# toybox-rs/Toybox

Hardware: NVIDIA B200
Metric: env-steps/sec with rendered frames (higher is better)
Workload: dtype f64+u8

## Files before the change

### toybox_b200/csrc/tbx_direct.cu

```cuda
#include <mutex>
#include "tbx_render_direct.cuh"
#include <stdlib.h>
#include <vector>

using namespace tbxk;

static int align16(int v) { return (v + 15) & ~15; }

template <class D> static cudaError_t upload_direct(const std::vector<D> &A, Buf<uint8_t> &aux) {
  return A[0].ok ? aux.upload(reinterpret_cast<const uint8_t *>(A.data()), sizeof(D)) : cudaSuccess;
}

cudaError_t tbx_direct_build(const tbx::Config &c, const BrkTable *brk_default, const tbx::ResizeTab &rs, const TbxAreaPlan &plan, const uint8_t *base0_gray,
                             Buf<uint8_t> &aux, Buf<uint8_t> &aux2) {
  if (c.game == TBX_BREAKOUT) {
    if (!brk_default) return cudaSuccess;
    std::vector<TbxBrkDirect> A(1);
    tbx::build_brk_direct(c, *brk_default, rs, plan, base0_gray, A[0]);
    return upload_direct(A, aux);
  }
  if (c.game == TBX_AMIDAR) {
    std::vector<TbxAmiDirect> A(1);
    tbx::build_ami_direct(c, rs, plan, A[0]);
    return upload_direct(A, aux);
  }
  std::vector<TbxSiDirect> A(1);
  std::vector<TbxSpritePatch> patches;
  tbx::build_si_direct(c, rs, plan, base0_gray, A[0], patches);
  const cudaError_t e = upload_direct(A, aux);
  if (e != cudaSuccess || !aux || patches.empty()) return e;
  return aux2.upload(reinterpret_cast<const uint8_t *>(patches.data()), patches.size() * sizeof(TbxSpritePatch));
}

template <class K> static cudaError_t persistent_grid(K kernel, int smem, int n_chunks, int *grid_out) {
  struct Entry { const void *k; int smem, dev, resident; };
  static Entry cache[64];
  static int n_cache = 0;
  static std::mutex mu;
  int dev = 0;
  cudaGetDevice(&dev);
  int resident = 0;
  {
    std::lock_guard<std::mutex> lock(mu);
    for (int i = 0; i < n_cache; i++)
      if (cache[i].k == (const void *)kernel && cache[i].smem == smem && cache[i].dev == dev) resident = cache[i].resident;
  }
  if (!resident) {
    int per_sm = 0, sms = 0;
    cudaError_t e = cudaOccupancyMaxActiveBlocksPerMultiprocessor(&per_sm, kernel, TBX_DIRECT_THREADS, smem);
    if (e != cudaSuccess) return e;
    cudaDeviceGetAttribute(&sms, cudaDevAttrMultiProcessorCount, dev);
    resident = (per_sm > 0 ? per_sm : 1) * (sms > 0 ? sms : 148);
    std::lock_guard<std::mutex> lock(mu);
    if (n_cache < 64) cache[n_cache++] = Entry{(const void *)kernel, smem, dev, resident};
  }
  int grid = n_chunks < resident ? n_chunks : resident;
  if (const char *env = getenv("TBX_DIRECT_GRID")) if (atoi(env) > 0) grid = atoi(env) < n_chunks ? atoi(env) : n_chunks;
  *grid_out = grid;
  return cudaSuccess;
}

template <class... P, class... A> static cudaError_t launch_persistent(void (*kernel)(P...), int smem, int n, cudaStream_t s, const A &...args) {
  cudaError_t e = cudaFuncSetAttribute(kernel, cudaFuncAttributeMaxDynamicSharedMemorySize, smem);
  if (e != cudaSuccess) return e;
  int grid = 1;
  e = persistent_grid(kernel, smem, (n + TBX_EPC - 1) / TBX_EPC, &grid);
  if (e != cudaSuccess) return e;
  kernel<<<grid, TBX_DIRECT_THREADS, smem, s>>>(args...);
  return cudaGetLastError();
}

cudaError_t tbx_launch_direct(const tbx::Config &c, const RenderArgs &a, const TbxAreaPlan &plan, DirectArgs d, cudaStream_t s) {
// ... 40 lines not shown
```

### toybox_b200/csrc/tbx_direct.h

```cpp
#ifndef TBX_DIRECT_H
#define TBX_DIRECT_H
#include "tbx_breakout.h"
#include "tbx_space_invaders.h"
#include "tbx_amidar.h"

struct TbxMover { int x0, y0, x1, y1; uint32_t gray; };

#define TBX_BD_MAX_STATIC 16
#define TBX_BD_MAX_CLS 8
#define BRK_N_MOVERS (1 + TBX_BRK_MAX_BALLS)
typedef struct TbxBrkDirect {
  int32_t ok;
  int32_t ncols, nrows;
  int32_t wx0, wy0, bw, bh;
  int32_t wdy0, wdy1;
  int32_t hud_dyhi;
  int32_t n_static, _pad;
  uint32_t paddle_gray, ball_gray;
  uint8_t xcol[TBX_AREA_MAX_SRC];
  uint8_t yrow[TBX_AREA_MAX_SRC];
  uint8_t col0[TBX_AREA_MAX_DST];
  uint8_t dyrows[TBX_AREA_MAX_DST];
  uint8_t hsel[TBX_AREA_MAX_DST][TBX_AREA_MAX_TAPS];
  uint32_t wordcols[32];
  uint8_t brickgray[TBX_BRK_MAX_BRICKS];
  uint32_t inv32[TBX_AREA_MAX_DST + 1];
  alignas(16) float hlut[TBX_BRK_MAX_ROWS][4][TBX_AREA_MAX_DST];
  alignas(16) float hstatic[TBX_BD_MAX_STATIC][TBX_AREA_MAX_DST];
  int32_t n_cls, _pad2[3];
  uint8_t rowcls[TBX_BRK_H];
  alignas(16) uint8_t clsrows[TBX_BD_MAX_CLS * TBX_BRK_W + 16];
} TbxBrkDirect;

TBX_HD TbxMover brk_mover(const uint32_t *R, const BrkCfg &c, uint32_t paddle_gray, uint32_t ball_gray, int m) {
  TbxMover v; v.x0 = v.y0 = v.x1 = v.y1 = 0; v.gray = m == 0 ? paddle_gray : ball_gray;
  if (m < 0 || m >= BRK_N_MOVERS) return v;
  const TbxPrim p = brk_prim(R, c, (const BrkTable *)0, m == 0 ? BRK_SLOT_PADDLE : BRK_SLOT_BALLS + m - 1);
  if (p.h <= 0) return v;
  const int x0 = p.x < 0 ? 0 : p.x, y0 = p.y < 0 ? 0 : p.y;
  const int x1 = p.x + p.w > TBX_BRK_W ? TBX_BRK_W : p.x + p.w, y1 = p.y + p.h > TBX_BRK_H ? TBX_BRK_H : p.y + p.h;
  if (x0 >= x1 || y0 >= y1) return v;
  v.x0 = x0; v.y0 = y0; v.x1 = x1; v.y1 = y1;
  return v;
}

TBX_HD uint32_t brk_col_bits(const uint32_t *alive, int nrows, int c) {
  const int i0 = c * nrows, w = i0 >> 5, s = i0 & 31;
  const uint32_t lo = alive[w], hi = w < 4 ? alive[w + 1] : 0u;
  const uint32_t v = s ? (lo >> s) | (hi << (32 - s)) : lo;
  return v & ((1u << nrows) - 1u);
}

TBX_HD uint32_t brk_direct_src(const TbxBrkDirect &A, const uint8_t *base0, const uint32_t *alive, const TbxMover *mv, uint32_t near, bool wall,
                               int x, int y) {
  uint32_t v = base0[y * TBX_BRK_W + x];
  if (wall) {
    const uint32_t c = A.xcol[x], r = A.yrow[y];
    if ((c | r) != 255u) {
      const uint32_t i = c * (uint32_t)A.nrows + r;
      if ((alive[i >> 5] >> (i & 31)) & 1u) v = A.brickgray[i];
    }
  }
#if defined(__CUDA_ARCH__)
#pragma unroll
#endif
  for (int m = 0; m < BRK_N_MOVERS; m++)
    if ((near >> m) & 1u)
      if ((unsigned)(x - mv[m].x0) < (unsigned)(mv[m].x1 - mv[m].x0) && (unsigned)(y - mv[m].y0) < (unsigned)(mv[m].y1 - mv[m].y0)) v = mv[m].gray;
  return v;
}

template <int TX, int TY>
TBX_HD uint8_t brk_direct_pixel(const TbxBrkDirect &A, const TbxAreaPlan &pl, const uint8_t *base0, const uint32_t *alive, const TbxMover *mv, uint32_t near,
                                bool wall, int dx, int dy) {
  const int xs = pl.xs0[dx], ys = pl.ys0[dy];
  float acc = 0.0f;
#if defined(__CUDA_ARCH__)
#pragma unroll
#endif
  for (int k = 0; k < TY; k++) {
    const int y = ys + k < TBX_BRK_H ? ys + k : TBX_BRK_H - 1;
    float h = 0.0f;
#if defined(__CUDA_ARCH__)
#pragma unroll
#endif
// ... 87 lines not shown
```

### toybox_b200/csrc/tbx_host.cpp

```cpp
#include "tbx_host.h"
#include "tbx_breakout.h"
#include "tbx_space_invaders.h"
#include "tbx_amidar.h"
#include "tbx_direct.h"
#include <errno.h>
#include <math.h>
#include <string.h>

using tbxjson::Value;

namespace tbx {

static void fail(const std::string &m) { throw std::runtime_error(m); }

static const GameInfo GAMES[3] = {
    {TBX_BREAKOUT, "breakout", TBX_BRK_W, TBX_BRK_H, 4, {0, 1, 3, 4}, TBX_WORDS(BrkRec), BRK_N_SLOTS, 2},
    {TBX_AMIDAR, "amidar", TBX_AMI_W, TBX_AMI_H, 10, {0, 1, 2, 3, 4, 5, 10, 11, 12, 13}, TBX_WORDS(AmiRec), AMI_N_SLOTS, 1},
    {TBX_SPACE_INVADERS, "space_invaders", TBX_SI_W, TBX_SI_H, 6, {0, 1, 3, 4, 11, 12}, TBX_WORDS(SiRec), SI_N_SLOTS, 2},
};
const GameInfo *game_info(int game) { return game >= 0 && game < 3 ? &GAMES[game] : 0; }
int game_from_name(const char *name) {
  if (!name) return -1;
  for (int g = 0; g < 3; g++) if (strcmp(GAMES[g].name, name) == 0) return g;
  if (strcmp(name, "spaceinvaders") == 0) return TBX_SPACE_INVADERS;
// ... 844 lines not shown
  for (int y = 0; y < H; y++) for (int dx = 0; dx < dw; dx++) buf[(size_t)y * dw + dx] = tbx_area_h(gray + (size_t)y * W, t.x, dx);
  for (int dy = 0; dy < dh; dy++) for (int dx = 0; dx < dw; dx++) out[dy * dw + dx] = tbx_area_v(buf.data(), dw, 0, t.y, dy, dx);
}
int digit_slot0(int game) { return game == TBX_BREAKOUT ? BRK_SLOT_SCORE : game == TBX_AMIDAR ? AMI_SLOT_SCORE : SI_SLOT_SCORE; }
int digit_slots(int game) { return game == TBX_BREAKOUT ? BRK_SLOT_BRICKS - BRK_SLOT_SCORE : game == TBX_AMIDAR ? AMI_N_SLOTS - AMI_SLOT_SCORE : SI_SLOT_SHIELDS - SI_SLOT_SCORE; }
static uint8_t area_pixel(const uint8_t *gray, int W, const ResizeTab &t, int dx, int dy) {
  int k = t.y.start[dy], k1 = t.y.start[dy + 1];
  float s = tbx_fmul(t.y.alpha[k], tbx_area_h(gray + (size_t)t.y.si[k] * W, t.x, dx));
  for (k++; k < k1; k++) s = tbx_fadd(s, tbx_fmul(t.y.alpha[k], tbx_area_h(gray + (size_t)t.y.si[k] * W, t.x, dx)));
  int v = tbx_f2i_rn(s);
  return (uint8_t)(v < 0 ? 0 : v > 255 ? 255 : v);
}
void build_digit_patches(const Config &c, const BrkTable *brk_default, const ResizeTab &t, const TbxAreaPlan &plan, const uint8_t *base_gray,
                         TbxDigitPatch *out) {
  const GameInfo *gi = game_info(c.game);
  const int W = gi->width, H = gi->height;
  std::vector<uint8_t> gray(base_gray, base_gray + (size_t)W * H);
  std::vector<uint32_t> rec(gi->rec_words, 0);
  memset(out, 0, sizeof(TbxDigitPatch) * TBX_DP_SLOTS * 10);
  const int s0 = digit_slot0(c.game), ns = digit_slots(c.game);
  for (int idx = 0; idx < ns && idx < TBX_DP_SLOTS; idx++) {
    const int k = idx % TBX_MAX_DIGITS;
    for (int d = 0; d < 10; d++) {
      long long v = d;
      for (int i = 0; i < k; i++) v *= 10;
      if (d == 0 && k > 0) { v = 1; for (int i = 0; i <= k; i++) v *= 10; }
      if (v > 2000000000LL) continue;
      std::fill(rec.begin(), rec.end(), 0u);
      TbxHdr &h = *reinterpret_cast<TbxHdr *>(rec.data());
      h.score = (int32_t)v; h.lives = (int32_t)v;
      TbxPrim p;
      if (c.game == TBX_BREAKOUT) p = brk_prim(rec.data(), c.brk, brk_default, s0 + idx);
      else if (c.game == TBX_AMIDAR) { reinterpret_cast<AmiRec *>(rec.data())->jumps = (int32_t)v; p = ami_prim(rec.data(), c.ami, 0, s0 + idx); }
      else { reinterpret_cast<SiRec *>(rec.data())->life_display_timer = 1; p = si_prim(rec.data(), s0 + idx); }
      if (p.h <= 0 || p.bw != 3 || p.off != TBX_BANK_FONT + 5 * d) continue;
      const int x0 = p.x < 0 ? 0 : p.x, x1 = p.x + p.w > W ? W : p.x + p.w, y0 = p.y < 0 ? 0 : p.y, y1 = p.y + p.h > H ? H : p.y + p.h;
      if (x0 >= x1 || y0 >= y1) continue;
      const int dx0 = plan.xdlo[x0], dx1 = plan.xdhi[x1 - 1], dy0 = plan.ydlo[y0], dy1 = plan.ydhi[y1 - 1];
      const int w = dx1 - dx0 + 1, hh = dy1 - dy0 + 1;
      if (w < 1 || hh < 1 || w > 8 || w * hh > TBX_DP_MAX) continue;
      const uint8_t lum = (uint8_t)tbx_luma(p.color);
      for (int y = y0; y < y1; y++)
        for (int x = x0; x < x1; x++)
          if (tbx_prim_covers(p, HOST_BANK, rec.data(), x, y)) gray[(size_t)y * W + x] = lum;
      TbxDigitPatch &P = out[idx * 10 + d];
      P.x0 = (uint8_t)dx0; P.y0 = (uint8_t)dy0; P.w = (uint8_t)w; P.h = (uint8_t)hh;
      for (int r = 0; r < hh; r++)
        for (int cc = 0; cc < w; cc++) P.px[r * w + cc] = area_pixel(gray.data(), W, t, dx0 + cc, dy0 + r);
      for (int y = y0; y < y1; y++) memcpy(&gray[(size_t)y * W + x0], base_gray + (size_t)y * W + x0, (size_t)(x1 - x0));
    }
  }
}

static float hsum_row(const uint8_t *row, int W, const TbxAreaPlan &pl, int dx) {
  float h = 0.0f;
  for (int t = 0; t < TBX_AREA_MAX_TAPS; t++) {
    const int x = pl.xs0[dx] + t < W ? pl.xs0[dx] + t : W - 1;
    const float p = tbx_fmul((float)row[x], pl.xalpha[t][dx]);
    h = t == 0 ? p : tbx_fadd(h, p);
  }
  return h;
}
void build_brk_direct(const Config &c, const BrkTable &t, const ResizeTab &rs, const TbxAreaPlan &pl, const uint8_t *base0, TbxBrkDirect &A) {
  memset(&A, 0, sizeof A);
  const int W = TBX_BRK_W, H = TBX_BRK_H, dw = pl.dw, dh = pl.dh;
  if (c.game != TBX_BREAKOUT || !t.delta_ok || dw % 4 != 0 || dw > TBX_AREA_MAX_DST || dh > TBX_AREA_MAX_DST || pl.tx > 5 || pl.ty > 4) return;
  const int n = t.n_bricks, nrows = c.brk.n_rows;
  if (n <= 0 || nrows <= 0 || nrows > TBX_BRK_MAX_ROWS || n % nrows != 0) return;
  const int ncols = n / nrows;
  if (ncols > 31) return;
  const int bw = t.iw[0], bh = t.ih[0], wx0 = t.ix[0], wy0 = t.iy[0];
  if (bw <= 0 || bh <= 0 || wx0 < 0 || wy0 < 0 || wx0 + ncols * bw > W || wy0 + nrows * bh > H) return;
  for (int i = 0; i < n; i++) {
    const int col = i / nrows, row = i % nrows;
    if (t.ix[i] != wx0 + col * bw || t.iy[i] != wy0 + row * bh || t.iw[i] != bw || t.ih[i] != bh) return;
    A.brickgray[i] = (uint8_t)tbx_luma(t.color[i]);
  }
  A.ncols = ncols; A.nrows = nrows; A.wx0 = wx0; A.wy0 = wy0; A.bw = bw; A.bh = bh;
  A.paddle_gray = tbx_luma(c.brk.paddle_color); A.ball_gray = tbx_luma(c.brk.ball_color);
  for (int k = 2; k <= TBX_AREA_MAX_DST; k++) A.inv32[k] = 0xffffffffu / (uint32_t)k + 1u;
  memset(A.xcol, 255, sizeof A.xcol);
  memset(A.yrow, 255, sizeof A.yrow);
  for (int x = wx0; x < wx0 + ncols * bw; x++) A.xcol[x] = (uint8_t)((x - wx0) / bw);
  for (int y = wy0; y < wy0 + nrows * bh; y++) A.yrow[y] = (uint8_t)((y - wy0) / bh);
  for (int r = 0; r < nrows; r++)
    for (int y = wy0 + r * bh + 1; y < wy0 + (r + 1) * bh; y++)
      if (memcmp(base0 + (size_t)y * W, base0 + (size_t)(wy0 + r * bh) * W, W) != 0) return;
  std::vector<uint8_t> row(W);
  for (int dx = 0; dx < dw; dx++) {
    int cmin = 255, cmax = -1;
    uint32_t cols = 0;
    for (int k = rs.x.start[dx]; k < rs.x.start[dx + 1]; k++) {
      const int cc = A.xcol[rs.x.si[k]];
      if (cc == 255) continue;
      cols |= 1u << cc;
      if (cc < cmin) cmin = cc;
      if (cc > cmax) cmax = cc;
    }
    if (cmax >= 0 && cmax - cmin > 1) return;
    int c0 = cmax < 0 ? 0 : cmin;
    if (c0 > ncols - 2) c0 = ncols - 2 < 0 ? 0 : ncols - 2;
    A.col0[dx] = (uint8_t)c0;
    A.wordcols[dx >> 2] |= cols;
    for (int r = 0; r < nrows; r++)
      for (int bits = 0; bits < 4; bits++) {
        memcpy(row.data(), base0 + (size_t)(wy0 + r * bh) * W, W);
        for (int j = 0; j < 2; j++) {
          const int cc = c0 + j;
          if (cc >= ncols || !((bits >> j) & 1)) continue;
          for (int x = wx0 + cc * bw; x < wx0 + (cc + 1) * bw; x++) row[x] = A.brickgray[cc * nrows + r];
        }
        A.hlut[r][bits][dx] = hsum_row(row.data(), W, pl, dx);
      }
  }
  const int wy1 = wy0 + nrows * bh;
  A.wdy0 = pl.ydlo[wy0]; A.wdy1 = pl.ydhi[wy1 - 1];
  if (A.wdy1 - A.wdy0 + 1 > 32) return;
  for (int dy = A.wdy0; dy <= A.wdy1; dy++) {
    const int nreal = rs.y.start[dy + 1] - rs.y.start[dy];
    for (int k = 0; k < TBX_AREA_MAX_TAPS; k++) {
      if (k >= nreal) { A.hsel[dy][k] = A.hsel[dy][0]; continue; }
      const int y = pl.ys0[dy] + k;
      if (A.yrow[y] != 255) { A.hsel[dy][k] = A.yrow[y]; A.dyrows[dy] |= (uint8_t)(1u << A.yrow[y]); continue; }
      float hrow[TBX_AREA_MAX_DST];
      for (int dx = 0; dx < dw; dx++) hrow[dx] = hsum_row(base0 + (size_t)y * W, W, pl, dx);
      int s = 0;
      for (; s < A.n_static; s++) if (memcmp(A.hstatic[s], hrow, sizeof(float) * dw) == 0) break;
      if (s == A.n_static) {
        if (A.n_static == TBX_BD_MAX_STATIC) return;
        memcpy(A.hstatic[A.n_static++], hrow, sizeof(float) * dw);
      }
      A.hsel[dy][k] = (uint8_t)(nrows + s);
    }
  }
  {
    std::vector<uint32_t> rec(TBX_WORDS(BrkRec), 0);
    TbxHdr &h = *reinterpret_cast<TbxHdr *>(rec.data());
    h.score = 1999999999; h.lives = 1999999999;
    int y1 = 0;
    for (int s = BRK_SLOT_SCORE; s < BRK_SLOT_BRICKS; s++) { const TbxPrim p = brk_prim(rec.data(), c.brk, &t, s); if (p.h > 0 && p.y + p.h > y1) y1 = p.y + p.h; }
    if (y1 > H) y1 = H;
    A.hud_dyhi = y1 > 0 ? pl.ydhi[y1 - 1] : -1;
    if (A.wdy0 <= A.hud_dyhi) return;
  }
  A.n_cls = 0;
  for (int y = 0; y < H; y++) {
    int cls = -1;
    for (int k = 0; k < A.n_cls && cls < 0; k++)
      if (memcmp(A.clsrows + (size_t)k * W, base0 + (size_t)y * W, W) == 0) cls = k;
    if (cls < 0) {
      if (A.n_cls == TBX_BD_MAX_CLS) { A.n_cls = 0; break; }
      cls = A.n_cls++;
      memcpy(A.clsrows + (size_t)cls * W, base0 + (size_t)y * W, W);
    }
    A.rowcls[y] = (uint8_t)cls;
  }
  A.ok = 1;
}

static void build_si_score_strip(const ResizeTab &rs, const TbxAreaPlan &pl, const uint8_t *base0, TbxSiDirect &A) {
  const int W = TBX_SI_W, H = TBX_SI_H;
  A.sc_ok = 0;
  A.sc_gray = (int32_t)tbx_luma(SI_COLOR_HUD);
  std::vector<uint32_t> rec(TBX_WORDS(SiRec), 0);
  TbxHdr &hd = *reinterpret_cast<TbxHdr *>(rec.data());
  int bx0[TBX_MAX_DIGITS], bx1[TBX_MAX_DIGITS], by0 = 0, by1 = 0;
  hd.score = 1999999999;
  for (int k = 0; k < TBX_MAX_DIGITS; k++) {
    const TbxPrim p = si_prim(rec.data(), SI_SLOT_SCORE + k);
    if (p.h <= 0 || p.bw != 3 || p.x < 0 || p.y < 0 || p.x + p.w > W || p.y + p.h > H) return;
    if (k > 0 && (p.y != by0 || p.y + p.h != by1 || p.x + p.w > bx0[k - 1])) return;
    bx0[k] = p.x; bx1[k] = p.x + p.w; by0 = p.y; by1 = p.y + p.h;
  }
  const int dx0 = pl.xdlo[bx0[TBX_MAX_DIGITS - 1]], dx1 = pl.xdhi[bx1[0] - 1], dy0 = pl.ydlo[by0], dy1 = pl.ydhi[by1 - 1];
  const int ncol = dx1 - dx0 + 1, nrow = dy1 - dy0 + 1;
  if (ncol < 1 || ncol > TBX_SC_MAX_COLS || nrow < 1 || nrow > TBX_SC_MAX_ROWS) return;
  std::vector<uint8_t> gray(base0, base0 + (size_t)W * H);
  const uint8_t lum = (uint8_t)A.sc_gray;
  for (int c = 0; c < ncol; c++) {
    const int dx = dx0 + c;
    int lo = -1, hi = -1;
    for (int k = 0; k < TBX_MAX_DIGITS; k++) {
      bool touch = false;
      for (int kx = rs.x.start[dx]; kx < rs.x.start[dx + 1]; kx++) touch |= rs.x.si[kx] >= bx0[k] && rs.x.si[kx] < bx1[k];
      if (touch) { if (lo < 0) lo = k; hi = k; }
    }
    if (hi > lo + 1) return;
    A.sc_slot[c] = lo < 0 ? 255 : (uint8_t)lo;
    for (int da = 0; da <= 10; da++)
      for (int db = 0; db <= 10; db++) {
        bool possible = lo >= 0 && da < 10 && !(db == 10 && da == 0 && lo > 0) && !(db < 10 && lo + 1 >= TBX_MAX_DIGITS);
        long long v = 0;
        if (possible) {
          long long pw = 1;
          for (int i = 0; i < lo; i++) pw *= 10;
          v = da * pw + (db < 10 ? db * pw * 10 : 0);
          if (db == 0) v += pw * 100;
          if (v > 2147483647LL) possible = false;
          if (db == 0 && lo + 2 >= TBX_MAX_DIGITS) possible = false;
        }
        if (possible) {
          hd.score = (int32_t)v;
          for (int k = lo; k <= lo + 1 && k < TBX_MAX_DIGITS; k++) {
            const TbxPrim p = si_prim(rec.data(), SI_SLOT_SCORE + k);
            if (p.h <= 0) continue;
            for (int y = p.y; y < p.y + p.h; y++)
              for (int x = p.x; x < p.x + p.w; x++)
                if (tbx_prim_covers(p, HOST_BANK, rec.data(), x, y)) gray[(size_t)y * W + x] = lum;
          }
        }
        for (int r = 0; r < nrow; r++) A.sc_px[c][da][db][r] = area_pixel(gray.data(), W, rs, dx, dy0 + r);
        if (possible)
          for (int y = by0; y < by1; y++) memcpy(&gray[(size_t)y * W + bx0[TBX_MAX_DIGITS - 1]], base0 + (size_t)y * W + bx0[TBX_MAX_DIGITS - 1], (size_t)(bx1[0] - bx0[TBX_MAX_DIGITS - 1]));
      }
  }
  A.sc_dx0 = dx0; A.sc_ncol = ncol; A.sc_dy0 = dy0; A.sc_nrow = nrow;
  A.sc_ok = 1;
}

static int gcd_int(int a, int b) { while (b) { int t = a % b; a = b; b = t; } return a; }
void build_si_direct(const Config &c, const ResizeTab &rs, const TbxAreaPlan &pl, const uint8_t *base0, TbxSiDirect &A, std::vector<TbxSpritePatch> &patches) {
  memset(&A, 0, sizeof A);
  patches.clear();
  const int W = TBX_SI_W, H = TBX_SI_H, dw = pl.dw, dh = pl.dh;
  if (c.game != TBX_SPACE_INVADERS || dw % 4 != 0 || dw > TBX_AREA_MAX_DST || dh > TBX_AREA_MAX_DST || pl.tx > 5 || pl.ty > 4) return;
  A.bg_gray = (int32_t)tbx_luma(SI_COLOR_BLACK);
  for (int dy = 0; dy < dh; dy++)
    for (int dx = 0; dx < dw; dx++) {
      bool plain = true;
      for (int ky = rs.y.start[dy]; ky < rs.y.start[dy + 1] && plain; ky++)
        for (int kx = rs.x.start[dx]; kx < rs.x.start[dx + 1]; kx++)
          if (base0[(size_t)rs.y.si[ky] * W + rs.x.si[kx]] != (uint8_t)A.bg_gray) { plain = false; break; }
      if (plain) A.plain[dy][dx >> 5] |= 1u << (dx & 31);
    }
  A.px_period = W / gcd_int(W, dw); A.ox_period = dw / gcd_int(W, dw);
  A.py_period = H / gcd_int(H, dh); A.oy_period = dh / gcd_int(H, dh);
  for (int k = 2; k <= TBX_AREA_MAX_DST; k++) A.inv32[k] = 0xffffffffu / (uint32_t)k + 1u;
  A.inv_px = A.px_period > 1 ? 0xffffffffu / (uint32_t)A.px_period + 1u : 0u;
  A.inv_py = A.py_period > 1 ? 0xffffffffu / (uint32_t)A.py_period + 1u : 0u;
  A.ok = 1;
  build_si_score_strip(rs, pl, base0, A);
  for (int dx = 0; dx + A.ox_period < dw; dx++) {
    if (pl.xs0[dx + A.ox_period] != pl.xs0[dx] + A.px_period) return;
    for (int t = 0; t < TBX_AREA_MAX_TAPS; t++) if (memcmp(&pl.xalpha[t][dx + A.ox_period], &pl.xalpha[t][dx], sizeof(float)) != 0) return;
  }
  for (int dy = 0; dy + A.oy_period < dh; dy++) {
    if (pl.ys0[dy + A.oy_period] != pl.ys0[dy] + A.py_period) return;
    for (int t = 0; t < TBX_AREA_MAX_TAPS; t++) if (memcmp(&pl.yalpha[t][dy + A.oy_period], &pl.yalpha[t][dy], sizeof(float)) != 0) return;
  }
  struct Set { int off, h; uint32_t color; };
  std::vector<Set> sets;
  for (int k = 0; k < 6; k++) sets.push_back({TBX_BANK_INVADER + 10 * k, SI_ENEMY_H, SI_COLOR_ENEMY});
  sets.push_back({TBX_BANK_BOOM, SI_ENEMY_H, SI_COLOR_ENEMY});
  sets.push_back({TBX_BANK_SHIP, SI_ENEMY_H, SI_COLOR_SHIP});
  sets.push_back({TBX_BANK_BOOM, SI_ENEMY_H, SI_COLOR_SHIP});
  sets.push_back({TBX_BANK_BOOM + 10, SI_ENEMY_H, SI_COLOR_SHIP});
  sets.push_back({TBX_BANK_UFO, SI_UFO_H, SI_COLOR_UFO});
  sets.push_back({TBX_BANK_BOOM + 10, SI_ENEMY_H, SI_COLOR_UFO});
  const size_t n_phase = (size_t)A.px_period * A.py_period;
  if (sets.size() > TBX_SD_MAX_SETS || n_phase * sets.size() * sizeof(TbxSpritePatch) > ((size_t)4 << 20)) return;
  std::vector<uint8_t> canvas((size_t)W * H);
  std::vector<TbxSpritePatch> out(n_phase * sets.size());
  for (size_t s = 0; s < sets.size(); s++) {
    const uint8_t g = (uint8_t)tbx_luma(sets[s].color);
    for (int yp = 0; yp < A.py_period; yp++)
      for (int xp = 0; xp < A.px_period; xp++) {
        int x = xp, y = yp;
        while (x + 16 > W) x -= A.px_period;
        while (y + sets[s].h > H) y -= A.py_period;
        if (x < 0 || y < 0) return;
        std::fill(canvas.begin(), canvas.end(), (uint8_t)A.bg_gray);
        for (int r = 0; r < sets[s].h; r++)
          for (int q = 0; q < 16; q++)
            if ((HOST_BANK[sets[s].off + r] >> (15 - q)) & 1u) canvas[(size_t)(y + r) * W + x + q] = g;
        const int dx0 = pl.xdlo[x], dx1 = pl.xdhi[x + 15], dy0 = pl.ydlo[y], dy1 = pl.ydhi[y + sets[s].h - 1];
        const int w = dx1 - dx0 + 1, h = dy1 - dy0 + 1;
        if (w > TBX_SP_MAX_W || h > TBX_SP_MAX_H) return;
        TbxSpritePatch &P = out[(s * A.py_period + yp) * A.px_period + xp];
        P.w = (uint8_t)w; P.h = (uint8_t)h;
        for (int r = 0; r < h; r++)
          for (int q = 0; q < w; q++) P.px[r * TBX_SP_MAX_W + q] = area_pixel(canvas.data(), W, rs, dx0 + q, dy0 + r);
      }
  }
  A.n_sets = (int32_t)sets.size();
  memset(A.set_lut, 255, sizeof A.set_lut);
  for (size_t s = 0; s < sets.size(); s++) {
    const int idx = sets[s].off >= TBX_BANK_BOOM ? 8 + (sets[s].off - TBX_BANK_BOOM) / 10 : (sets[s].off - TBX_BANK_INVADER) / 10;
    for (int k = 0; k < 4; k++) if (A.set_lut[idx][k] == 255) { A.set_lut[idx][k] = (uint8_t)s; break; }
  }
  for (size_t s = 0; s < sets.size(); s++) { A.set_off[s] = (uint16_t)sets[s].off; A.set_gray[s] = (uint8_t)tbx_luma(sets[s].color); A.set_h[s] = (uint8_t)sets[s].h; }
  patches.swap(out);
}

void build_ami_direct(const Config &c, const ResizeTab &rs, const TbxAreaPlan &pl, TbxAmiDirect &A) {
  memset(&A, 0, sizeof A);
  const int W = TBX_AMI_W, H = TBX_AMI_H, dw = pl.dw, dh = pl.dh;
  if (c.game != TBX_AMIDAR || dw % 4 != 0 || dw > TBX_AREA_MAX_DST || dh > TBX_AREA_MAX_DST || pl.tx > 4 || pl.ty > 4) return;
  const AmiCfg &cf = c.ami;
  A.gray[0] = tbx_luma(cf.bg_color); A.gray[1] = tbx_luma(cf.unpainted_color); A.gray[2] = tbx_luma(cf.painted_color); A.gray[3] = tbx_luma(cf.inner_painted_color);
  A.player_gray = tbx_luma(cf.player_color); A.enemy_gray = tbx_luma(cf.enemy_color);
  for (int ty = 0; ty < TBX_AMI_BH; ty++) for (int k = 0; k < 2; k++) A.base_looks[ty][k] = ami_looks_of_tags(cf.board[ty][k]);
  for (int k = 2; k <= TBX_AREA_MAX_DST; k++) A.inv32[k] = 0xffffffffu / (uint32_t)k + 1u;
  memset(A.xcol, 255, sizeof A.xcol);
  memset(A.yrow, 255, sizeof A.yrow);
  const int mx0 = AMI_OFF_X, mx1 = AMI_OFF_X + 4 * TBX_AMI_BW, my0 = AMI_OFF_Y, my1 = AMI_OFF_Y + 5 * TBX_AMI_BH;
  if (mx1 > W || my1 > H) return;
  for (int x = mx0; x < mx1; x++) A.xcol[x] = (uint8_t)((x - mx0) / 4);
  for (int y = my0; y < my1; y++) A.yrow[y] = (uint8_t)((y - my0) / 5);
  std::vector<uint8_t> row(W);
  for (int dx = 0; dx < dw; dx++) {
    int cmin = 255, cmax = -1;
    for (int k = rs.x.start[dx]; k < rs.x.start[dx + 1]; k++) {
      const int cc = A.xcol[rs.x.si[k]];
      if (cc == 255) continue;
      A.wordcols[dx >> 2][cc >> 4] |= 3u << (2 * (cc & 15));
      if (cc < cmin) cmin = cc;
      if (cc > cmax) cmax = cc;
    }
    if (cmax >= 0 && cmax - cmin > 1) return;
    int c0 = cmax < 0 ? 0 : cmin;
    if (c0 > TBX_AMI_BW - 2) c0 = TBX_AMI_BW - 2;
    A.col0[dx] = (uint8_t)c0;
    for (int idx = 0; idx < 16; idx++) {
      std::fill(row.begin(), row.end(), (uint8_t)A.gray[0]);
      for (int j = 0; j < 2; j++) {
        const int look = (idx >> (2 * j)) & 3;
        for (int x = mx0 + 4 * (c0 + j); x < mx0 + 4 * (c0 + j + 1); x++) row[x] = (uint8_t)A.gray[look];
      }
      A.hlut[idx][dx] = hsum_row(row.data(), W, pl, dx);
    }
  }
  A.mdy0 = pl.ydlo[my0]; A.mdy1 = pl.ydhi[my1 - 1];
  for (int dy = 0; dy < dh; dy++) {
    const int nreal = rs.y.start[dy + 1] - rs.y.start[dy];
    for (int k = 0; k < TBX_AREA_MAX_TAPS; k++) {
// ... 22 lines not shown
```

### toybox_b200/csrc/tbx_host.h

```cpp
#ifndef TBX_HOST_H
#define TBX_HOST_H
#include "tbx_records.h"
#include "tbx_json.h"
#include <string>
#include <vector>

struct TbxBrkDirect;
struct TbxSiDirect;
struct TbxAmiDirect;
struct TbxSpritePatch;

namespace tbx {

struct GameInfo {
  int id;
  const char *name;
  int width, height;
  int n_legal;
  int legal[18];
  int rec_words;
  int n_slots;
  int new_games_at_ctor;
};
const GameInfo *game_info(int game);
int game_from_name(const char *name);

struct Config {
  int game;
  BrkCfg brk;
  SiCfg si;
  AmiCfg ami;
};
void default_config(int game, Config &c);
void brk_finish_cfg(BrkCfg &c);
tbxjson::Value config_to_json(const Config &c);
void config_from_json(Config &c, const tbxjson::Value &v);

void brk_default_table(const BrkCfg &c, BrkTable &t);
void brk_finish_table(BrkTable &t);
void ami_default_table(const AmiCfg &c, AmiTable &t);
void ami_finish_table(AmiTable &t);

tbxjson::Value brk_state_to_json(const BrkRec &r, const BrkTable &t);
void brk_state_from_json(const tbxjson::Value &v, BrkRec &r, BrkTable &t);
tbxjson::Value si_state_to_json(const SiRec &r);
void si_state_from_json(const tbxjson::Value &v, SiRec &r);
tbxjson::Value ami_state_to_json(const AmiRec &r, const AmiTable &t);
void ami_state_from_json(const tbxjson::Value &v, AmiRec &r, AmiTable &t);

tbxjson::Value query_json(int game, const uint32_t *rec, const BrkTable *brk, const std::string &query, const tbxjson::Value &args);

tbxjson::Value schema_for_state(int game);
tbxjson::Value schema_for_config(int game);

typedef TbxResizeAxis ResizeAxis;
typedef TbxResizeTab ResizeTab;
void build_resize(int sw, int sh, int dw, int dh, ResizeTab &t);
bool build_area_plan(const ResizeTab &t, TbxAreaPlan &plan);

int n_static_slots(int game);
void build_base_frame(const Config &c, const BrkTable *brk_default, int base_id, uint32_t *rgba);
void brk_mark_delta_ok(const Config &c, BrkTable &t);
void frame_to_gray(const uint32_t *rgba, int npix, uint8_t *gray);
void area_resize(const uint8_t *gray, const ResizeTab &t, uint8_t *out);
void build_digit_patches(const Config &c, const BrkTable *brk_default, const ResizeTab &t, const TbxAreaPlan &plan, const uint8_t *base_gray,
                         TbxDigitPatch *out);
void build_brk_direct(const Config &c, const BrkTable &t, const ResizeTab &rs, const TbxAreaPlan &plan, const uint8_t *base0_gray, TbxBrkDirect &out);
void build_si_direct(const Config &c, const ResizeTab &rs, const TbxAreaPlan &plan, const uint8_t *base0_gray, TbxSiDirect &out, std::vector<TbxSpritePatch> &patches);
void build_ami_direct(const Config &c, const ResizeTab &rs, const TbxAreaPlan &plan, TbxAmiDirect &out);
int digit_slot0(int game);
int digit_slots(int game);

}
#endif
```

### toybox_b200/csrc/tbx_render_direct.cuh

```cuda
#ifndef TBX_RENDER_DIRECT_CUH
#define TBX_RENDER_DIRECT_CUH
#include "tbx_render_area.cuh"
#include "tbx_direct.h"
#include "tbx_direct_launch.h"

namespace tbxk {

#define TBX_DIRECT_THREADS 256
#define TBX_BRK_DIG_SLOTS 6
#define TBX_BRK_DIG_WORDS 13
#define TBX_BRK_DIG_BYTES (TBX_BRK_DIG_SLOTS * 10 * TBX_BRK_DIG_WORDS * 4)
__host__ __device__ __forceinline__ int brk_plan_pitch(int dw, int dh) { return ((dw > dh ? dw : dh) + 3) & ~3; }
__host__ __device__ __forceinline__ int brk_plan_smem_bytes(int tx, int ty, int dw, int dh) { return ((tx + ty) * brk_plan_pitch(dw, dh) * 4 + 2 * brk_plan_pitch(dw, dh) * 2 + 15) & ~15; }
__host__ __device__ __forceinline__ int si_tab_smem_bytes(int dw, int dh) { return ((dh * ((dw + 31) >> 5) + 3) & ~3) * 4 + ((TBX_AREA_MAX_DST + 1 + 3) & ~3) * 4; }
__host__ __device__ __forceinline__ int ami_tab_smem_bytes(int dh) { return TBX_AMI_W + 256 + ((dh * 4 + 15) & ~15); }
__device__ __forceinline__ int brk_dig_cid(int slot) { return slot < 4 ? slot : slot >= TBX_MAX_DIGITS && slot < TBX_MAX_DIGITS + 2 ? slot - TBX_MAX_DIGITS + 4 : -1; }
#define TBX_BRK_TAB_BYTES (TBX_BRK_DIG_BYTES + TBX_BD_MAX_CLS * TBX_BRK_W + 16 + TBX_BRK_H + (TBX_AREA_MAX_DST + 1 + 3) / 4 * 16)
#ifndef TBX_DIRECT_MIN_CTAS
#define TBX_DIRECT_MIN_CTAS 4
#endif

__device__ __forceinline__ void cp_async16(void *smem_dst, const void *gsrc) {
  asm volatile("cp.async.cg.shared.global [%0], [%1], 16;" ::"r"((uint32_t)__cvta_generic_to_shared(smem_dst)), "l"(gsrc) : "memory");
}
// ... 79 lines not shown
  const int ok = A.ok, ncols = A.ncols, nrows = A.nrows, wdy0 = A.wdy0, wdy1 = A.wdy1, hud_dyhi = A.hud_dyhi;
  const int wy0 = A.wy0, wy1 = A.wy0 + A.nrows * A.bh;
  const uint32_t paddle_gray = A.paddle_gray, ball_gray = A.ball_gray;
  const TbxDigitPatch *__restrict__ patches = a.patches[1];
  __syncthreads();
  const bool dig_smem = s_bigdig == 0;
  const uint32_t *R = recw;

  int st = 0, it = 0, nxt = 0;
  for (int chunk = (int)blockIdx.x * 2 + team; chunk < n_chunks; chunk = nxt, st ^= 1, it++) {
    cp_async_wait_all();
    asm volatile("bar.sync %0, %1;" ::"r"(1 + team), "r"(TEAM_THREADS) : "memory");
    nxt = s_next[team][it & 1];
    if (nxt < n_chunks) prefetch(nxt, st ^ 1);
    if (ttid == 0) s_next[team][(it + 1) & 1] = n_teams + atomicAdd(d.sched, 1);
    const int env = chunk * TEAM + wt;
    if (env >= a.n) continue;
    {
      const uint32_t *src = tstage + st * RW * TEAM + wt;
      for (int w = lane; w < RW; w += 32) recw[w] = src[w * TEAM];
    }
    __syncwarp();
    uint8_t *out = a.dst + (size_t)env * a.env_stride + (size_t)a.stack_slot * a.frame_bytes;
    const TbxMover mine = brk_mover(R, cfg_c, paddle_gray, ball_gray, lane < BRK_N_MOVERS ? lane : -1);
    const bool valid = mine.x0 < mine.x1;
    int fx0 = 0, fx1 = 0, fy0 = 0, fy1 = 0;
    if (valid) { fx0 = __ldg(&plan->xdlo[mine.x0]); fx1 = __ldg(&plan->xdhi[mine.x1 - 1]); fy0 = __ldg(&plan->ydlo[mine.y0]); fy1 = __ldg(&plan->ydhi[mine.y1 - 1]); }
    bool bad = valid && fy0 <= hud_dyhi;
    int dig = -1;
    const TbxDigitPatch *P = patches;
    if (lane < 2 * TBX_MAX_DIGITS && patches) {
      const int field = lane >= TBX_MAX_DIGITS;
      dig = tbx_digit_at((int32_t)R[field ? TBX_HW(lives) : TBX_HW(score)], lane - field * TBX_MAX_DIGITS);
      if (dig >= 0) {
        const int cid = brk_dig_cid(lane);
        P = patches + lane * 10 + dig;
        bad |= (dig_smem && cid >= 0 ? (sdig[(cid * 10 + dig) * TBX_BRK_DIG_WORDS] >> 16) & 255u : (uint32_t)__ldg(&P->w)) == 0;
      }
    }
    const bool covered = ok && patches && (int32_t)R[TBX_HW(tbl)] == cfg_c.default_tbl;
    if (!covered || __any_sync(0xffffffffu, bad)) {
      if (lane == 0) d.fb_list[atomicAdd(d.fb_count, 1)] = env;
      continue;
    }
    if (bulk) {
      if (lane == 0) {
        asm volatile("cp.async.bulk.global.shared::cta.bulk_group [%0], [%1], %2;" ::"l"(out), "r"((uint32_t)__cvta_generic_to_shared(sbase)), "r"((uint32_t)nb) : "memory");
        asm volatile("cp.async.bulk.commit_group;" ::: "memory");
      }
    } else {
      for (int i = lane; i < (nb >> 2); i += 32) reinterpret_cast<uint32_t *>(out)[i] = reinterpret_cast<const uint32_t *>(sbase)[i];
    }
    const uint32_t vm = __ballot_sync(0xffffffffu, valid) & ((1u << BRK_N_MOVERS) - 1u);
    if (lane < BRK_N_MOVERS) {
      const int ncol = valid ? fx1 - fx0 + 1 : 0, nrow = valid ? fy1 - fy0 + 1 : 0;
      mrec[3 * lane + 0] = make_int4(mine.x0, mine.y0, mine.x1, mine.y1);
      mrec[3 * lane + 1] = make_int4((int)mine.gray * 0x01010101, fx0, fy0, ncol);
      mrec[3 * lane + 2] = make_int4(ncol * nrow, ncol > 1 ? (int)sinv[ncol] : 0, 0, 0);
    }
    __syncwarp();
    int total = 0;
#pragma unroll
    for (int m = 0; m < BRK_N_MOVERS; m++) total += mrec[3 * m + 2].x;
    const uint32_t *__restrict__ base0w = reinterpret_cast<const uint32_t *>(a.base[0]);
    const uint32_t *alive = R + BRK_W(alive);
    auto mover_pixel = [&](int p0, int &o) -> uint32_t {
      const int l = p0 + lane;
      int mym = 0, myi = 0, off = 0;
#pragma unroll
      for (int m = 0; m < BRK_N_MOVERS; m++) {
        const int cnt = mrec[3 * m + 2].x;
        if (l >= off && l < off + cnt) { mym = m; myi = l - off; }
        off += cnt;
      }
      const bool act = l < total;
      const int4 f = mrec[3 * mym + 1];
      const int ncol = f.w, inv = mrec[3 * mym + 2].y;
      const int q = ncol > 1 ? (int)__umulhi((unsigned)myi, (unsigned)inv) : myi;
      const int dx = act ? f.y + myi - q * ncol : 0, dy = act ? f.z + q : 0;
      o = act ? dy * dw + dx : -1;
      const int xs = sxs[dx], ys = sys[dy];
      uint32_t lo[TY], hi[TY];
#pragma unroll
      for (int k = 0; k < TY; k++) {
        const int y = min(ys + k, TBX_BRK_H - 1);
        const uint32_t *rowp = n_cls ? reinterpret_cast<const uint32_t *>(scls + (int)srowcls[y] * TBX_BRK_W) : base0w + y * (TBX_BRK_W / 4);
        const uint32_t w0 = rowp[xs >> 2], w1 = rowp[(xs >> 2) + 1];
        lo[k] = __funnelshift_r(w0, w1, 8 * (xs & 3));
        hi[k] = 0;
        if (TX > 4) { const uint32_t w2 = rowp[(xs >> 2) + 2]; hi[k] = __funnelshift_r(w1, w2, 8 * (xs & 3)) & 255u; }
      }
      if (__any_sync(0xffffffffu, act && ys < wy1 && ys + TY > wy0)) {
        uint32_t cb[TX];
#pragma unroll
        for (int t = 0; t < TX; t++) cb[t] = __ldg(&A.xcol[min(xs + t, TBX_BRK_W - 1)]);
#pragma unroll
        for (int k = 0; k < TY; k++) {
          const uint32_t r = __ldg(&A.yrow[min(ys + k, TBX_BRK_H - 1)]);
          if (r == 255u) continue;
#pragma unroll
          for (int t = 0; t < TX; t++) {
            if (cb[t] == 255u) continue;
            const uint32_t i = cb[t] * (uint32_t)nrows + r;
            if (!((alive[i >> 5] >> (i & 31)) & 1u)) continue;
            const uint32_t g = __ldg(&A.brickgray[i]);
            if (t < 4) lo[k] = (lo[k] & ~(255u << (8 * t))) | (g << (8 * t));
            else hi[k] = g;
          }
        }
      }
      uint32_t mleft = vm;
      while (mleft) {
        const int m = __ffs(mleft) - 1;
        mleft &= mleft - 1;
        const int4 rc = mrec[3 * m];
        const uint32_t g4 = (uint32_t)mrec[3 * m + 1].x;
        const int ta = max(rc.x - xs, 0), tb = min(rc.z - xs, TX), ka = max(rc.y - ys, 0), kb = min(rc.w - ys, TY);
        if (ta >= tb || ka >= kb) continue;
        const uint32_t below_b = tb >= 4 ? 0xffffffffu : (1u << (8 * tb)) - 1u, below_a = ta >= 4 ? 0xffffffffu : (1u << (8 * ta)) - 1u;
        const uint32_t bm = below_b & ~below_a;
        const bool h5 = TX > 4 && ta <= 4 && tb > 4;
#pragma unroll
        for (int k = 0; k < TY; k++)
          if (k >= ka && k < kb) {
            lo[k] = (lo[k] & ~bm) | (g4 & bm);
            if (h5) hi[k] = g4 & 255u;
          }
      }
      float al[TX];
#pragma unroll
      for (int t = 0; t < TX; t++) al[t] = sxa[t * ps + dx];
      float acc = 0.0f;
#pragma unroll
// ... 762 lines not shown
```

Before: 470.7 million.

## Precompute phase-indexed paddle/ball patches for Breakout direct renderer

Adds host-built per-phase patches of the downscaled paddle and ball drawn on a plain background, plus a per-output-pixel plain mask. When a mover sits entirely over plain background and does not overlap another mover, the kernel reads the precomputed patch pixel instead of running the multi-tap area filter. This shares the periodicity check with the Space Invaders patch builder. It adds extra validation work per mover and a global patch lookup, and falls back to the full filter when any lane in the warp is not covered.

```diff
diff --git a/toybox_b200/csrc/tbx_direct.cu b/toybox_b200/csrc/tbx_direct.cu
--- a/toybox_b200/csrc/tbx_direct.cu
+++ b/toybox_b200/csrc/tbx_direct.cu
@@ -16,8 +16,12 @@
   if (c.game == TBX_BREAKOUT) {
     if (!brk_default) return cudaSuccess;
     std::vector<TbxBrkDirect> A(1);
+    std::vector<TbxMoverPatch> patches;
     tbx::build_brk_direct(c, *brk_default, rs, plan, base0_gray, A[0]);
-    return upload_direct(A, aux);
+    tbx::build_brk_mover_patches(c, *brk_default, rs, plan, base0_gray, A[0], patches);
+    const cudaError_t e = upload_direct(A, aux);
+    if (e != cudaSuccess || !aux || patches.empty()) return e;
+    return aux2.upload(reinterpret_cast<const uint8_t *>(patches.data()), patches.size() * sizeof(TbxMoverPatch));
   }
   if (c.game == TBX_AMIDAR) {
     std::vector<TbxAmiDirect> A(1);
diff --git a/toybox_b200/csrc/tbx_direct.h b/toybox_b200/csrc/tbx_direct.h
--- a/toybox_b200/csrc/tbx_direct.h
+++ b/toybox_b200/csrc/tbx_direct.h
@@ -30,7 +30,13 @@
   int32_t n_cls, _pad2[3];
   uint8_t rowcls[TBX_BRK_H];
   alignas(16) uint8_t clsrows[TBX_BD_MAX_CLS * TBX_BRK_W + 16];
+  int32_t n_sets, px_period, py_period, _pad3;
+  uint32_t inv_px, inv_py;
+  int32_t set_w[2], set_h[2];
+  uint32_t plain[TBX_AREA_MAX_DST][4];
 } TbxBrkDirect;
+#define TBX_MP_MAX_PX 46
+typedef struct TbxMoverPatch { uint8_t w, h; uint8_t px[TBX_MP_MAX_PX]; } TbxMoverPatch;
 
 TBX_HD TbxMover brk_mover(const uint32_t *R, const BrkCfg &c, uint32_t paddle_gray, uint32_t ball_gray, int m) {
   TbxMover v; v.x0 = v.y0 = v.x1 = v.y1 = 0; v.gray = m == 0 ? paddle_gray : ball_gray;
diff --git a/toybox_b200/csrc/tbx_host.cpp b/toybox_b200/csrc/tbx_host.cpp
--- a/toybox_b200/csrc/tbx_host.cpp
+++ b/toybox_b200/csrc/tbx_host.cpp
@@ -920,6 +920,38 @@
   }
 }
 
+static int gcd_int(int a, int b) { while (b) { int t = a % b; a = b; b = t; } return a; }
+static bool area_periods(const TbxAreaPlan &pl, int W, int H, int &px, int &py, int &ox, int &oy) {
+  const int dw = pl.dw, dh = pl.dh;
+  px = W / gcd_int(W, dw); ox = dw / gcd_int(W, dw);
+  py = H / gcd_int(H, dh); oy = dh / gcd_int(H, dh);
+  for (int dx = 0; dx + ox < dw; dx++) {
+    if (pl.xs0[dx + ox] != pl.xs0[dx] + px) return false;
+    for (int t = 0; t < TBX_AREA_MAX_TAPS; t++) if (memcmp(&pl.xalpha[t][dx + ox], &pl.xalpha[t][dx], sizeof(float)) != 0) return false;
+  }
+  for (int dy = 0; dy + oy < dh; dy++) {
+    if (pl.ys0[dy + oy] != pl.ys0[dy] + py) return false;
+    for (int t = 0; t < TBX_AREA_MAX_TAPS; t++) if (memcmp(&pl.yalpha[t][dy + oy], &pl.yalpha[t][dy], sizeof(float)) != 0) return false;
+  }
+  return true;
+}
+template <class Paint, class Store>
+static bool build_phase_patches(const ResizeTab &rs, const TbxAreaPlan &pl, int W, int H, int px, int py, int sw, int sh, uint8_t bg, Paint paint, Store store) {
+  std::vector<uint8_t> canvas((size_t)W * H);
+  for (int yp = 0; yp < py; yp++)
+    for (int xp = 0; xp < px; xp++) {
+      int x = xp, y = yp;
+      while (x + sw > W) x -= px;
+      while (y + sh > H) y -= py;
+      if (x < 0 || y < 0) return false;
+      std::fill(canvas.begin(), canvas.end(), bg);
+      paint(canvas.data(), x, y);
+      const int dx0 = pl.xdlo[x], dx1 = pl.xdhi[x + sw - 1], dy0 = pl.ydlo[y], dy1 = pl.ydhi[y + sh - 1];
+      if (!store(xp, yp, dx1 - dx0 + 1, dy1 - dy0 + 1, [&](int c, int r) { return area_pixel(canvas.data(), W, rs, dx0 + c, dy0 + r); })) return false;
+    }
+  return true;
+}
+
 static float hsum_row(const uint8_t *row, int W, const TbxAreaPlan &pl, int dx) {
   float h = 0.0f;
   for (int t = 0; t < TBX_AREA_MAX_TAPS; t++) {
@@ -1024,6 +1056,57 @@
     A.rowcls[y] = (uint8_t)cls;
   }
   A.ok = 1;
+}
+void build_brk_mover_patches(const Config &c, const BrkTable &t, const ResizeTab &rs, const TbxAreaPlan &pl, const uint8_t *base0, TbxBrkDirect &A,
+                             std::vector<TbxMoverPatch> &patches) {
+  patches.clear();
+  A.n_sets = 0;
+  memset(A.plain, 0, sizeof A.plain);
+  if (!A.ok) return;
+  const int W = TBX_BRK_W, H = TBX_BRK_H, dw = pl.dw, dh = pl.dh;
+  const uint8_t bg = (uint8_t)tbx_luma(c.brk.bg_color);
+  for (int dy = A.hud_dyhi + 1; dy < dh; dy++)
+    for (int dx = 0; dx < dw; dx++) {
+      bool plain = true;
+      for (int ky = rs.y.start[dy]; ky < rs.y.start[dy + 1] && plain; ky++)
+        for (int kx = rs.x.start[dx]; kx < rs.x.start[dx + 1]; kx++) {
+          const int x = rs.x.si[kx], y = rs.y.si[ky];
+          if (base0[(size_t)y * W + x] != bg || (A.xcol[x] != 255 && A.yrow[y] != 255)) { plain = false; break; }
+        }
+      if (plain) A.plain[dy][dx >> 5] |= 1u << (dx & 31);
+    }
+  int pxp = 1, pyp = 1, oxp = 1, oyp = 1;
+  if (!area_periods(pl, W, H, pxp, pyp, oxp, oyp)) return;
+  std::vector<uint32_t> rec(TBX_WORDS(BrkRec), 0);
+  TbxAcc S; S.p = rec.data(); S.stride = 1;
+  brk_new_game(S, c.brk);
+  S.sti(BRK_W(n_balls), 1);
+  const TbxPrim sp[2] = {brk_prim(rec.data(), c.brk, &t, BRK_SLOT_PADDLE), brk_prim(rec.data(), c.brk, &t, BRK_SLOT_BALLS)};
+  const size_t n_phase = (size_t)pxp * pyp;
+  if (n_phase * 2 * sizeof(TbxMoverPatch) > ((size_t)4 << 20)) return;
+  std::vector<TbxMoverPatch> out(n_phase * 2);
+  for (int s = 0; s < 2; s++) {
+    const int sw = sp[s].w, sh = sp[s].h;
+    const uint8_t g = (uint8_t)(s == 0 ? A.paddle_gray : A.ball_gray);
+    if (sp[s].h <= 0 || sw <= 0 || sw > W || sh > H) return;
+    const bool ok = build_phase_patches(rs, pl, W, H, pxp, pyp, sw, sh, bg,
+      [&](uint8_t *canvas, int x, int y) { for (int r = 0; r < sh; r++) memset(canvas + (size_t)(y + r) * W + x, g, (size_t)sw); },
+      [&](int xp, int yp, int w, int h, auto pixel) {
+        if (w * h > TBX_MP_MAX_PX) return false;
+        TbxMoverPatch &P = out[((size_t)s * pyp + yp) * pxp + xp];
+        P.w = (uint8_t)w; P.h = (uint8_t)h;
+        for (int r = 0; r < h; r++)
+          for (int q = 0; q < w; q++) P.px[r * w + q] = pixel(q, r);
+        return true;
+      });
+    if (!ok) return;
+    A.set_w[s] = sw; A.set_h[s] = sh;
+  }
+  A.px_period = pxp; A.py_period = pyp;
+  A.inv_px = pxp > 1 ? 0xffffffffu / (uint32_t)pxp + 1u : 0u;
+  A.inv_py = pyp > 1 ? 0xffffffffu / (uint32_t)pyp + 1u : 0u;
+  A.n_sets = 2;
+  patches.swap(out);
 }
 
 static void build_si_score_strip(const ResizeTab &rs, const TbxAreaPlan &pl, const uint8_t *base0, TbxSiDirect &A) {
@@ -1086,7 +1169,6 @@
   A.sc_ok = 1;
 }
 
-static int gcd_int(int a, int b) { while (b) { int t = a % b; a = b; b = t; } return a; }
 void build_si_direct(const Config &c, const ResizeTab &rs, const TbxAreaPlan &pl, const uint8_t *base0, TbxSiDirect &A, std::vector<TbxSpritePatch> &patches) {
   memset(&A, 0, sizeof A);
   patches.clear();
@@ -1101,21 +1183,15 @@
           if (base0[(size_t)rs.y.si[ky] * W + rs.x.si[kx]] != (uint8_t)A.bg_gray) { plain = false; break; }
       if (plain) A.plain[dy][dx >> 5] |= 1u << (dx & 31);
     }
-  A.px_period = W / gcd_int(W, dw); A.ox_period = dw / gcd_int(W, dw);
-  A.py_period = H / gcd_int(H, dh); A.oy_period = dh / gcd_int(H, dh);
+  int pxp = 1, pyp = 1, oxp = 1, oyp = 1;
+  const bool periodic = area_periods(pl, W, H, pxp, pyp, oxp, oyp);
+  A.px_period = pxp; A.py_period = pyp; A.ox_period = oxp; A.oy_period = oyp;
   for (int k = 2; k <= TBX_AREA_MAX_DST; k++) A.inv32[k] = 0xffffffffu / (uint32_t)k + 1u;
   A.inv_px = A.px_period > 1 ? 0xffffffffu / (uint32_t)A.px_period + 1u : 0u;
   A.inv_py = A.py_period > 1 ? 0xffffffffu / (uint32_t)A.py_period + 1u : 0u;
   A.ok = 1;
   build_si_score_strip(rs, pl, base0, A);
-  for (int dx = 0; dx + A.ox_period < dw; dx++) {
-    if (pl.xs0[dx + A.ox_period] != pl.xs0[dx] + A.px_period) return;
-    for (int t = 0; t < TBX_AREA_MAX_TAPS; t++) if (memcmp(&pl.xalpha[t][dx + A.ox_period], &pl.xalpha[t][dx], sizeof(float)) != 0) return;
-  }
-  for (int dy = 0; dy + A.oy_period < dh; dy++) {
-    if (pl.ys0[dy + A.oy_period] != pl.ys0[dy] + A.py_period) return;
-    for (int t = 0; t < TBX_AREA_MAX_TAPS; t++) if (memcmp(&pl.yalpha[t][dy + A.oy_period], &pl.yalpha[t][dy], sizeof(float)) != 0) return;
-  }
+  if (!periodic) return;
   struct Set { int off, h; uint32_t color; };
   std::vector<Set> sets;
   for (int k = 0; k < 6; k++) sets.push_back({TBX_BANK_INVADER + 10 * k, SI_ENEMY_H, SI_COLOR_ENEMY});
@@ -1127,28 +1203,25 @@
   sets.push_back({TBX_BANK_BOOM + 10, SI_ENEMY_H, SI_COLOR_UFO});
   const size_t n_phase = (size_t)A.px_period * A.py_period;
   if (sets.size() > TBX_SD_MAX_SETS || n_phase * sets.size() * sizeof(TbxSpritePatch) > ((size_t)4 << 20)) return;
-  std::vector<uint8_t> canvas((size_t)W * H);
   std::vector<TbxSpritePatch> out(n_phase * sets.size());
   for (size_t s = 0; s < sets.size(); s++) {
     const uint8_t g = (uint8_t)tbx_luma(sets[s].color);
-    for (int yp = 0; yp < A.py_period; yp++)
-      for (int xp = 0; xp < A.px_period; xp++) {
-        int x = xp, y = yp;
-        while (x + 16 > W) x -= A.px_period;
-        while (y + sets[s].h > H) y -= A.py_period;
-        if (x < 0 || y < 0) return;
-        std::fill(canvas.begin(), canvas.end(), (uint8_t)A.bg_gray);
-        for (int r = 0; r < sets[s].h; r++)
+    const Set &S = sets[s];
+    const bool ok = build_phase_patches(rs, pl, W, H, A.px_period, A.py_period, 16, S.h, (uint8_t)A.bg_gray,
+      [&](uint8_t *canvas, int x, int y) {
+        for (int r = 0; r < S.h; r++)
           for (int q = 0; q < 16; q++)
-            if ((HOST_BANK[sets[s].off + r] >> (15 - q)) & 1u) canvas[(size_t)(y + r) * W + x + q] = g;
-        const int dx0 = pl.xdlo[x], dx1 = pl.xdhi[x + 15], dy0 = pl.ydlo[y], dy1 = pl.ydhi[y + sets[s].h - 1];
-        const int w = dx1 - dx0 + 1, h = dy1 - dy0 + 1;
-        if (w > TBX_SP_MAX_W || h > TBX_SP_MAX_H) return;
+            if ((HOST_BANK[S.off + r] >> (15 - q)) & 1u) canvas[(size_t)(y + r) * W + x + q] = g;
+      },
+      [&](int xp, int yp, int w, int h, auto pixel) {
+        if (w > TBX_SP_MAX_W || h > TBX_SP_MAX_H) return false;
         TbxSpritePatch &P = out[(s * A.py_period + yp) * A.px_period + xp];
         P.w = (uint8_t)w; P.h = (uint8_t)h;
         for (int r = 0; r < h; r++)
-          for (int q = 0; q < w; q++) P.px[r * TBX_SP_MAX_W + q] = area_pixel(canvas.data(), W, rs, dx0 + q, dy0 + r);
-      }
+          for (int q = 0; q < w; q++) P.px[r * TBX_SP_MAX_W + q] = pixel(q, r);
+        return true;
+      });
+    if (!ok) return;
   }
   A.n_sets = (int32_t)sets.size();
   memset(A.set_lut, 255, sizeof A.set_lut);
diff --git a/toybox_b200/csrc/tbx_host.h b/toybox_b200/csrc/tbx_host.h
--- a/toybox_b200/csrc/tbx_host.h
+++ b/toybox_b200/csrc/tbx_host.h
@@ -9,6 +9,7 @@
 struct TbxSiDirect;
 struct TbxAmiDirect;
 struct TbxSpritePatch;
+struct TbxMoverPatch;
 
 namespace tbx {
 
@@ -66,6 +67,8 @@
 void build_digit_patches(const Config &c, const BrkTable *brk_default, const ResizeTab &t, const TbxAreaPlan &plan, const uint8_t *base_gray,
                          TbxDigitPatch *out);
 void build_brk_direct(const Config &c, const BrkTable &t, const ResizeTab &rs, const TbxAreaPlan &plan, const uint8_t *base0_gray, TbxBrkDirect &out);
+void build_brk_mover_patches(const Config &c, const BrkTable &t, const ResizeTab &rs, const TbxAreaPlan &plan, const uint8_t *base0_gray, TbxBrkDirect &out,
+                             std::vector<TbxMoverPatch> &patches);
 void build_si_direct(const Config &c, const ResizeTab &rs, const TbxAreaPlan &plan, const uint8_t *base0_gray, TbxSiDirect &out, std::vector<TbxSpritePatch> &patches);
 void build_ami_direct(const Config &c, const ResizeTab &rs, const TbxAreaPlan &plan, TbxAmiDirect &out);
 int digit_slot0(int game);
diff --git a/toybox_b200/csrc/tbx_render_direct.cuh b/toybox_b200/csrc/tbx_render_direct.cuh
--- a/toybox_b200/csrc/tbx_render_direct.cuh
+++ b/toybox_b200/csrc/tbx_render_direct.cuh
@@ -155,13 +155,44 @@
       for (int i = lane; i < (nb >> 2); i += 32) reinterpret_cast<uint32_t *>(out)[i] = reinterpret_cast<const uint32_t *>(sbase)[i];
     }
     const uint32_t vm = __ballot_sync(0xffffffffu, valid) & ((1u << BRK_N_MOVERS) - 1u);
+    const TbxMoverPatch *__restrict__ mpatch = reinterpret_cast<const TbxMoverPatch *>(d.aux2);
     if (lane < BRK_N_MOVERS) {
       const int ncol = valid ? fx1 - fx0 + 1 : 0, nrow = valid ? fy1 - fy0 + 1 : 0;
+      int pidx = -1;
+      const int s = lane ? 1 : 0;
+      if (valid && A.n_sets && mine.x1 - mine.x0 == A.set_w[s] && mine.y1 - mine.y0 == A.set_h[s]) {
+        const int pxp = A.px_period, pyp = A.py_period;
+        const uint32_t ipx = A.inv_px, ipy = A.inv_py, ox = (uint32_t)mine.x0, oy = (uint32_t)mine.y0;
+        const uint32_t xph = ipx ? ox - __umulhi(ox, ipx) * (uint32_t)pxp : 0u, yph = ipy ? oy - __umulhi(oy, ipy) * (uint32_t)pyp : 0u;
+        const int idx = (s * pyp + (int)yph) * pxp + (int)xph;
+        const uint32_t wh = __ldg(reinterpret_cast<const uint16_t *>(mpatch + idx));
+        bool ok = (int)(wh & 255u) == ncol && (int)(wh >> 8) == nrow;
+        for (int r = fy0; r <= fy1 && ok; r++)
+          for (int w = fx0 >> 5; w <= fx1 >> 5; w++) {
+            const uint32_t mask = (w == fx0 >> 5 ? 0xffffffffu << (fx0 & 31) : 0xffffffffu) & (w == fx1 >> 5 ? 0xffffffffu >> (31 - (fx1 & 31)) : 0xffffffffu);
+            ok &= (__ldg(&A.plain[r][w]) & mask) == mask;
+          }
+        if (ok) pidx = idx;
+      }
       mrec[3 * lane + 0] = make_int4(mine.x0, mine.y0, mine.x1, mine.y1);
       mrec[3 * lane + 1] = make_int4((int)mine.gray * 0x01010101, fx0, fy0, ncol);
-      mrec[3 * lane + 2] = make_int4(ncol * nrow, ncol > 1 ? (int)sinv[ncol] : 0, 0, 0);
-    }
-    __syncwarp();
+      mrec[3 * lane + 2] = make_int4(ncol * nrow, ncol > 1 ? (int)sinv[ncol] : 0, nrow, pidx);
+    }
+    __syncwarp();
+    if (vm & (vm - 1)) {
+      if (lane < BRK_N_MOVERS && mrec[3 * lane + 2].w >= 0) {
+        bool alone = true;
+#pragma unroll
+        for (int q = 0; q < BRK_N_MOVERS; q++)
+          if (q != lane && ((vm >> q) & 1u)) {
+            const int4 f = mrec[3 * q + 1];
+            const int nr = mrec[3 * q + 2].z;
+            if (f.y <= fx1 && f.y + f.w > fx0 && f.z <= fy1 && f.z + nr > fy0) alone = false;
+          }
+        if (!alone) mrec[3 * lane + 2].w = -1;
+      }
+      __syncwarp();
+    }
     int total = 0;
 #pragma unroll
     for (int m = 0; m < BRK_N_MOVERS; m++) total += mrec[3 * m + 2].x;
@@ -177,11 +208,12 @@
         off += cnt;
       }
       const bool act = l < total;
-      const int4 f = mrec[3 * mym + 1];
-      const int ncol = f.w, inv = mrec[3 * mym + 2].y;
+      const int4 f = mrec[3 * mym + 1], g = mrec[3 * mym + 2];
+      const int ncol = f.w, inv = g.y;
       const int q = ncol > 1 ? (int)__umulhi((unsigned)myi, (unsigned)inv) : myi;
       const int dx = act ? f.y + myi - q * ncol : 0, dy = act ? f.z + q : 0;
       o = act ? dy * dw + dx : -1;
+      if (!__any_sync(0xffffffffu, act && g.w < 0)) return act ? (uint32_t)__ldg(&mpatch[g.w].px[myi]) : 0u;
       const int xs = sxs[dx], ys = sys[dy];
       uint32_t lo[TY], hi[TY];
 #pragma unroll
```

Result: slower. 422.0 million, median of 6 (-10.3%).
